# AroneyS/galah

Measured on AMD Instinct MI355X. Metric: precluster genome-pairs/sec at 10k genomes (s=1000) + sketch Gbases/s, higher is better.
Workload: dtype u64; 1 GPU; C3: 10000 synthetic genomes x 3000000 bp, clusters of 10, sub rate U(0,0.07), k=21, s=1000, min_ani=0.95; genomes=10000, genome_len=3000000, sketch_size=1000, k=21, parallelism=dp1, mode=lib

## Files before the change

galah_amd/csrc/api.cpp:

```cpp
#include <hip/hip_runtime.h>

#include <algorithm>
#include <chrono>
#include <cmath>
#include <cstdio>
#include <cstdlib>
#include <cstring>
#include <map>
#include <mutex>
#include <new>
#include <string>
#include <thread>
#include <vector>

#include "context.hpp"


namespace gg {

thread_local std::string g_thread_err;

void set_thread_error(const std::string& msg) { g_thread_err = msg; }

gg_status fail(gg_ctx* c, gg_status st, const std::string& msg) {
// ... 705 lines not shown
  b.border = n_old != 0;
  b.border0 = n_old;
  const char* re = getenv("GALAHGPU_INDEX_RANGE");
  const bool range_on = !(re && *re == '0');
  if (range_on && (r0 > 0 || r1 < n) && 5ull * (r1 - r0) <= 2ull * n) {
    uint32_t lg = 20;
    while (lg < 30 && (1ull << lg) < 16ull * (r1 - r0) * c->s) ++lg;
    b.bloom_log2 = lg;
    b.r0 = r0;
    b.r1 = r1;
    GG_HIP(c, scratch_t(c, "idx_bloom", (size_t)1 << (lg - 5), &b.bloom));
  }
  const char* be = getenv("GALAHGPU_INDEX_BUCKETS");
  b.bucket = !(be && *be == '0');
  if (b.bucket) {
    GG_HIP(c, scratch_t(c, "idx_hist", kIndexCoarse, &b.hist));
    GG_HIP(c, scratch_t(c, "idx_bbase", kIndexCoarse + 1, &b.bbase));
  }
  IndexLaunch a;
  a.sketches = d_sk;
  a.lens = d_lens;
  a.n = n;
  a.stride = c->s;
  a.kbits = kbits;
  a.row0 = r0;
  a.nb = nb;
  a.tile_begin = tb;
  a.tile_end = te;
  a.runinfo = b.runinfo;
  a.vals = b.keys_in;
  a.cmin = d_cmin;
  a.sufmin = d_sufmin;
  a.tmax = 2 * c->s;
  a.out = d_out;
  a.out_cap = cap;
  a.count = (unsigned long long*)d_count;
  a.border = n_old != 0;
  {
    const char* e = getenv("GALAHGPU_INDEX_MAX_SPLIT");
    a.max_split_log2 = e && *e ? (uint32_t)std::min(16, std::max(0, atoi(e))) : 16u;
  }
  a.overflow = b.flags + 2;
  {
    const char* e = getenv("GALAHGPU_INDEX_COST");
    const double k = !weigh_cost ? 0.0 : e && *e ? atof(e) : 0.0;
    const uint64_t n_new = n - n_old;
    const uint64_t npairs = n_old ? n_new * n_old + n_new * (n_new - 1) / 2 : pairs_in_tiles(n, tb, te);
    const double lim = k * (double)c->s * (double)npairs;
    a.cost = b.cost;
    a.cost_limit = k > 0 && lim < 1.8e19 ? (unsigned long long)lim : ~0ull;
  }
  uint64_t* d_count0;
  GG_HIP(c, scratch_t(c, "idx_count0", 1, &d_count0));
  GG_HIP(c, hipMemcpyAsync(d_count0, d_count, sizeof(uint64_t), hipMemcpyDeviceToDevice, st));
  auto launch_pairs = [&](bool guarded) -> gg_status {
    a.build_flags = guarded ? b.flags : nullptr;
    a.ents16 = b.bucket && index_ents16(n);
    GG_HIP(c, timed_launch(c, GG_KERNEL_PAIRS, work, st, [&] { return launch_index_pairs(a, r1 - r0, st); }));
    return GG_OK;
  };
  uint64_t info[2] = {0, 0};
  uint32_t kept = 0;
  uint32_t flags[4] = {0, 0, 0, 0};
  bool built = false, paired = false;
  if (b.bucket && !b.bloom) {
    const uint32_t nbb = index_bucket_bound(total);
    const char* se = getenv("GALAHGPU_INDEX_SPLIT");
    const bool split = !(se && *se == '0');
    if (split) {
      GG_HIP(c, scratch_t(c, "idx_split_cnt", (size_t)256 * n + 1, &b.split_cnt));
      GG_HIP(c, scratch_t(c, "idx_split_off", (size_t)256 * n + 1, &b.split_off));
      GG_HIP(c, scratch_t(c, "idx_split_hist", (size_t)256 * 16 * 256, &b.split_hist));
    }
    b.sort_tmp_bytes = split ? index_split_tmp_bytes(n) : index_bucket_sort_tmp_bytes(total);
    GG_HIP(c, scratch(c, "idx_sort_tmp", b.sort_tmp_bytes, &b.sort_tmp));
    GG_HIP(c, scratch_t(c, "idx_bstart", split ? (size_t)65537 : (size_t)nbb + 1, &b.bstart));
    GG_HIP(c, timed_launch(c, GG_KERNEL_PAIRS_INDEX, total, st, [&] { return index_fill(b, st); }));
    GG_HIP(c, timed_launch(c, GG_KERNEL_PAIRS_INDEX, 0, st, [&] { return index_build_buckets(b, total, nbb, st); }));
    gg_status ps = launch_pairs(true);
    if (ps != GG_OK) return ps;
    uint64_t* h_if;
    GG_HIP(c, host_scratch_t(c, "idx_info", 5, &h_if));
    GG_HIP(c, hipMemcpyAsync(h_if, b.info, 5 * sizeof(uint64_t), hipMemcpyDeviceToHost, st));
    GG_HIP(c, hipStreamSynchronize(st));
    memcpy(info, h_if, sizeof info);
    memcpy(flags, h_if + 2, sizeof flags);
    built = paired = flags[3] == 0;
    if (built && !flags[0] && h_if[4] > a.cost_limit) {
      *costly = true;
      return GG_OK;
    }
  } else {
    uint32_t nbuckets = 0;
    GG_HIP(c, timed_launch(c, GG_KERNEL_PAIRS_INDEX, total, st, [&] { return index_fill(b, st); }));
    GG_HIP(c, hipMemcpyAsync(info, b.info, sizeof info, hipMemcpyDeviceToHost, st));
    if (b.bloom) GG_HIP(c, hipMemcpyAsync(&kept, b.flags + 1, sizeof kept, hipMemcpyDeviceToHost, st));
    if (b.bucket)
      GG_HIP(c, hipMemcpyAsync(&nbuckets, b.bbase + kIndexCoarse, sizeof nbuckets, hipMemcpyDeviceToHost, st));
    GG_HIP(c, hipStreamSynchronize(st));
    if (b.bucket) {
      b.sort_tmp_bytes = index_bucket_sort_tmp_bytes(kept);
      GG_HIP(c, scratch(c, "idx_sort_tmp", b.sort_tmp_bytes, &b.sort_tmp));
      GG_HIP(c, scratch_t(c, "idx_bstart", (size_t)nbuckets + 1, &b.bstart));
      GG_HIP(c, timed_launch(c, GG_KERNEL_PAIRS_INDEX, 0, st,
                             [&] { return index_build_buckets(b, kept, nbuckets, st); }));
      GG_HIP(c, hipMemcpyAsync(flags, b.flags, sizeof flags, hipMemcpyDeviceToHost, st));
      GG_HIP(c, hipStreamSynchronize(st));
// ... 745 lines not shown
```

galah_amd/csrc/gg_internal.hpp:

```cpp
#pragma once

#include <hip/hip_runtime.h>

#include <cstdint>
#include <memory>
#include <string>
#include <vector>

#include "../../include/galahgpu.h"

namespace gg {

constexpr uint64_t kEmpty = ~0ull;

enum SketchStatus : uint32_t {
  kSketchOk = 0,
  kSketchRetryLarger = 1,
  kSketchRetrySmaller = 2,
  kSketchRetrySet = 3,
};

constexpr uint32_t kFlagOverflow = 1u;
constexpr uint32_t kFlagSawMax = 2u;
constexpr uint32_t kFlagSetMode = 4u;
// ... 232 lines not shown
  const uint64_t* file_text;
  const uint64_t* unit_len;
  const uint64_t* unit_pad;
  const uint32_t* unit_lane;
  uint32_t n_lanes, n_units;
  uint8_t* text;
  uint16_t* sym;
  uint32_t* flags;
  uint64_t* prof = nullptr;
};
constexpr uint16_t kSymPtr = 0x8000u;
struct GzMember {
  uint64_t off = 0, len = 0;
  uint32_t isize = 0, crc = 0;
};
struct InflateFile {
  uint64_t data_off = 0, data_len = 0;
  uint32_t isize = 0, crc = 0;
  bool gz = false;
  std::vector<GzMember> members;
};
bool bgzf_members(const uint8_t* buf, uint64_t n, uint64_t base, std::vector<GzMember>& out);
uint64_t bgzf_member_size(const uint8_t* b, uint64_t n);
bool gzip_member(const uint8_t* buf, size_t n, size_t* data_off, size_t* data_len, uint32_t* isize, uint32_t* crc);
bool gzip_header(const uint8_t* buf, size_t n, uint64_t file_size, size_t* data_off);
hipError_t launch_inflate_search(const InflateSearch& a, hipStream_t st);
hipError_t launch_slot_upload(uint8_t* dst, const uint8_t* src_mapped, uint64_t bytes, hipStream_t st);
hipError_t launch_inflate_decode(const InflateDecode& a, hipStream_t st);
hipError_t launch_inflate_expand(const InflatePlace& a, hipStream_t st);
hipError_t launch_inflate_resolve(const InflatePlace& a, hipStream_t st);
constexpr uint32_t kInflateCrcSeg = 4096;
hipError_t launch_inflate_crc(const uint8_t* text, uint32_t n_files, const uint64_t* file_text, const uint64_t* file_len,
                              const uint32_t* seg_first, uint32_t n_segs, uint32_t* seg_crc, uint32_t* crc,
                              hipStream_t st);

struct IndexBuild {
  const uint64_t* sketches;
  const uint32_t* lens;
  uint32_t n;
  uint32_t stride;
  uint32_t kbits;
  uint32_t max_run;
  uint64_t* offs;
  uint64_t* info;
  uint32_t* keys_in;
  uint32_t* keys_out;
  uint64_t* vals_in;
  uint64_t* vals_out;
  uint64_t* runinfo;
  uint32_t* mixed;
  void* sort_tmp;
  size_t sort_tmp_bytes;
  uint32_t* flags;
  unsigned long long* cost;
  uint32_t* bloom = nullptr;
  uint32_t bloom_log2 = 0;
  uint32_t r0 = 0, r1 = 0;
  bool bucket = false;
  uint32_t* hist = nullptr;
  uint32_t* bbase = nullptr;
  uint32_t* bstart = nullptr;
  uint32_t* split_cnt = nullptr;
  uint32_t* split_off = nullptr;
  uint32_t* split_hist = nullptr;
  bool border = false;
  uint32_t border0 = 0;
};
struct IndexLaunch {
  const uint64_t* sketches;
  const uint32_t* lens;
  uint32_t n;
  uint32_t stride;
  uint32_t kbits;
  uint32_t row0;
  uint32_t n_rows;
  uint64_t nb;
  uint64_t tile_begin;
  uint64_t tile_end;
  const uint64_t* runinfo;
  const uint32_t* vals;
  const uint32_t* cmin;
  const uint32_t* sufmin;
  uint32_t tmax;
  gg_pair* out;
  uint64_t out_cap;
  unsigned long long* count;
  uint32_t max_split_log2;
  uint32_t* overflow;
  const uint32_t* build_flags = nullptr;
  bool ents16 = false;
  const unsigned long long* cost = nullptr;
  unsigned long long cost_limit = ~0ull;
  bool big_map = false;
  bool border = false;
};
hipError_t index_fill(const IndexBuild& b, hipStream_t st);
hipError_t index_build(const IndexBuild& b, uint64_t total, uint32_t sh, uint32_t end_bit, hipStream_t st);
hipError_t index_build_buckets(const IndexBuild& b, uint64_t total, uint32_t nb_bound, hipStream_t st);
uint32_t index_bucket_bound(uint64_t entries);
size_t index_cost_bytes();
size_t index_sort_tmp_bytes(uint64_t total, uint32_t end_bit);
size_t index_bucket_sort_tmp_bytes(uint64_t total);
size_t index_split_tmp_bytes(uint32_t n);
constexpr uint32_t kIndexCoarse = 4096;
hipError_t launch_index_pairs(const IndexLaunch& a, uint32_t n_rows, hipStream_t st);
bool index_ents16(uint32_t n);
// ... 60 lines not shown
```

galah_amd/csrc/pairs_index.hip:

```cpp
#include <hipcub/hipcub.hpp>

#include <algorithm>

#include "device_util.hpp"
#include "gg_internal.hpp"

namespace gg {
namespace {

constexpr int kRowThreads = 256;
constexpr int kScanThreads = 1024;
constexpr uint32_t kXcds = 8;

struct KeyShape {
  uint32_t sh, norm;
};
__device__ __forceinline__ KeyShape key_shape(unsigned long long maxh) {
  const uint32_t bits = maxh ? 64u - (uint32_t)__builtin_clzll(maxh) : 0u;
  const uint32_t sh = bits > 32 ? bits - 32 : 0u;
  const uint32_t eb = bits - sh > 1u ? bits - sh : 1u;
  return KeyShape{sh, 32u - eb};
}

constexpr uint32_t kCoarseBits = 12;
constexpr uint32_t kBucketPad = 0xFFFFu;
constexpr uint32_t kBucketKeyBits = 16;
constexpr uint32_t kCoarse = 1u << kCoarseBits;
__device__ __forceinline__ uint32_t bucket_of(uint64_t h, KeyShape ks, const uint32_t* __restrict__ bbase) {
  const uint32_t key = (uint32_t)(h >> ks.sh) << ks.norm;
  const uint32_t c = key >> (32 - kCoarseBits);
  const uint32_t rel = key & ((1u << (32 - kCoarseBits)) - 1u);
  const uint32_t b0 = bbase[c], ns = bbase[c + 1] - b0;
  return b0 + (uint32_t)(((uint64_t)rel * ns) >> (32 - kCoarseBits));
}

__device__ __forceinline__ uint32_t count_le(const uint64_t* __restrict__ a, uint32_t n, uint64_t x) {
  uint32_t lo = 0, hi = n;
  while (lo < hi) {
    const uint32_t mid = (lo + hi) >> 1;
    if (a[mid] <= x) lo = mid + 1;
    else hi = mid;
  }
  return lo;
}

__global__ __launch_bounds__(kScanThreads) void index_scan_kernel(const uint64_t* __restrict__ sk,
                                                                  const uint32_t* __restrict__ lens, uint32_t n,
                                                                  uint32_t stride, uint64_t* __restrict__ offs,
                                                                  unsigned long long* __restrict__ info) {
  __shared__ unsigned long long wsum[kScanThreads / 64], wmax[kScanThreads / 64];
  const uint32_t tid = threadIdx.x;
  const uint32_t per = (n + kScanThreads - 1) / kScanThreads;
  const uint32_t b0 = min(tid * per, n), b1 = min(b0 + per, n);
  unsigned long long sum = 0, mx = 0;
  for (uint32_t i = b0; i < b1; ++i) {
    const uint32_t l = lens[i];
    sum += l;
    if (l) mx = max(mx, (unsigned long long)sk[(uint64_t)i * stride + l - 1]);
  }
  unsigned long long inc = sum;
  for (int o = 1; o < 64; o <<= 1) {
    const unsigned long long y = __shfl_up(inc, o);
    if ((tid & 63) >= (uint32_t)o) inc += y;
  }
  for (int o = 32; o > 0; o >>= 1) mx = max(mx, (unsigned long long)__shfl_xor(mx, o));
  if ((tid & 63) == 63) wsum[tid >> 6] = inc;
  if ((tid & 63) == 0) wmax[tid >> 6] = mx;
  __syncthreads();
  unsigned long long run = inc - sum;
  for (uint32_t w = 0; w < (tid >> 6); ++w) run += wsum[w];
  for (uint32_t i = b0; i < b1; ++i) {
    offs[i] = run;
    run += lens[i];
  }
  if (tid == kScanThreads - 1) {
    info[0] = run;
    unsigned long long m = 0;
    for (int w = 0; w < kScanThreads / 64; ++w) m = max(m, wmax[w]);
    info[1] = m;
  }
}

template <bool BUCKET>
__global__ __launch_bounds__(256) void index_fill_kernel(const uint64_t* __restrict__ sk,
                                                         const uint32_t* __restrict__ lens,
                                                         const uint64_t* __restrict__ offs, uint32_t n,
                                                         uint32_t stride, uint32_t kbits, uint32_t sh,
                                                         const unsigned long long* __restrict__ info,
                                                         const uint32_t* __restrict__ bbase,
                                                         uint32_t* __restrict__ keys, uint64_t* __restrict__ vals) {
  const KeyShape ks = BUCKET ? key_shape(info[1]) : KeyShape{sh, 0u};
  for (uint32_t i = blockIdx.x; i < n; i += gridDim.x) {
    const uint32_t len = lens[i];
    const uint64_t* row = sk + (uint64_t)i * stride;
    if (BUCKET) {
      const uint64_t o = (uint64_t)i * stride;
      for (uint32_t k = threadIdx.x; k < stride; k += 256) {
        ((uint16_t*)keys)[o + k] = (uint16_t)(k < len ? bucket_of(row[k], ks, bbase) : kBucketPad);
        ((uint32_t*)vals)[o + k] = (i << kbits) | k;
      }
      continue;
    }
    const uint64_t o = offs[i];
    for (uint32_t k = threadIdx.x; k < len; k += 256) {
// ... 735 lines not shown
      uint32_t rk = rank[r];
      bool sorted_run = false;
      if (g >= 2 && g <= kRowSortedRun) {
        const uint32_t row = e >> kbits;
        rk = 0;
        for (uint32_t x = 0; x < g; ++x) rk += (grp[start + x] >> kbits) < row ? 1u : 0u;
        sorted_run = true;
      }
      if (ents16) ((uint16_t*)ents)[lo + start + rk] = (uint16_t)(e >> kbits);
      else ents[lo + start + rk] = e;
      if (g > max_run) {
        atomicOr(&flags[0], 1u);
        continue;
      }
      if (BEFORE) {
        const uint32_t cnt = g < 2 ? 0u : sorted_run ? rk : g;
        runinfo[(uint64_t)(e >> kbits) * stride + (e & kmask)] = run_reads((uint64_t)lo + start, cnt);
        if ((e >> kbits) >= border0) {
          reads += cnt;
          gmax = max(gmax, g);
        }
        continue;
      }
      const uint32_t cnt = g < 2 ? 0u : sorted_run ? g - 1u - rk : g;
      runinfo[(uint64_t)(e >> kbits) * stride + (e & kmask)] =
          run_reads((uint64_t)lo + start + (sorted_run ? rk + 1u : 0u), cnt);
      reads += cnt;
      gmax = max(gmax, g);
    }
  }
  cost_add(cost, reads, gmax);
}

__device__ __forceinline__ void row_columns(uint32_t i, uint32_t n, uint64_t nb, uint64_t tb, uint64_t te,
                                            uint32_t& jlo, uint32_t& jhi) {
  const uint64_t I = i / GG_PAIR_TILE;
  const uint64_t rs = I * nb - I * (I - 1) / 2;
  const uint64_t t0 = rs, t1 = rs + (nb - I);
  const uint64_t a = max(t0, tb), b = min(t1, te);
  if (a >= b) {
    jlo = jhi = 0;
    return;
  }
  const uint64_t J0 = I + (a - rs), J1 = I + (b - rs);
  jlo = (uint32_t)max<uint64_t>(J0 * GG_PAIR_TILE, (uint64_t)i + 1);
  jhi = (uint32_t)min<uint64_t>(J1 * GG_PAIR_TILE, (uint64_t)n);
}

__device__ __forceinline__ uint32_t part_of(uint32_t j, uint32_t plog2) {
  return plog2 ? (j * 0x9E3779B1u) >> (32 - plog2) : 0u;
}

constexpr uint32_t kMemberLoads = 8;
template <bool E16, uint32_t MAPLOG2, bool BORDER = false>
__global__ __launch_bounds__(kRowThreads) void index_pairs_kernel(IndexLaunch a) {
  constexpr uint32_t kMapLog2 = MAPLOG2, kMap = 1u << kMapLog2, kMapFull = kMap * 3 / 4;
  __shared__ uint32_t mkey[kMap];
  __shared__ uint32_t mcnt[kMap];
  __shared__ uint32_t fill;
  __shared__ volatile uint32_t over;
  const uint32_t tid = threadIdx.x;
  const uint32_t per_xcd = (a.n_rows + kXcds - 1) / kXcds;
  const uint32_t ri_ = (blockIdx.x % kXcds) * per_xcd + blockIdx.x / kXcds;
  if (ri_ >= a.n_rows) return;
  const uint32_t i = a.row0 + ri_;
  if (i >= a.n) return;
  if (a.build_flags && ((a.build_flags[0] | a.build_flags[3]) || (a.cost && *a.cost > a.cost_limit))) return;
  uint32_t jlo, jhi;
  if (BORDER) jlo = 0u, jhi = i;
  else row_columns(i, a.n, a.nb, a.tile_begin, a.tile_end, jlo, jhi);
  const uint32_t la = a.lens[i];
  if (jlo >= jhi || la == 0) return;
  const uint64_t* ri = a.runinfo + (uint64_t)i * a.stride;
  const uint64_t* A = a.sketches + (uint64_t)i * a.stride;
  const uint64_t xa = A[la - 1];
  uint32_t plog2 = 0;
  for (uint32_t p = 0; p < (1u << plog2);) {
    for (uint32_t x = tid; x < kMap; x += kRowThreads) mkey[x] = 0u, mcnt[x] = 0u;
    if (tid == 0) fill = 0u, over = 0u;
    __syncthreads();
    uint64_t info_next = tid < la ? ri[tid] : 0ull;
    for (uint32_t k = tid; k < la; k += kRowThreads) {
      if (over) break;
      const uint64_t info = info_next;
      info_next = k + kRowThreads < la ? ri[k + kRowThreads] : 0ull;
      const uint32_t cnt = (uint32_t)(info >> 32);
      if (cnt == 0) continue;
      const uint32_t q_first = (uint32_t)info, end = q_first + cnt;
      bool stop = false;
      for (uint32_t q0 = q_first; q0 < end && !stop; q0 += kMemberLoads) {
        uint32_t jv[kMemberLoads];
#pragma unroll
        for (uint32_t u = 0; u < kMemberLoads; ++u) {
          const uint32_t q = q0 + u;
          jv[u] = q < end ? (E16 ? (uint32_t)((const uint16_t*)a.vals)[q] : a.vals[q] >> a.kbits) : jhi;
        }
#pragma unroll
        for (uint32_t u = 0; u < kMemberLoads; ++u) {
          const uint32_t j = jv[u];
          if (stop || j < jlo || j >= jhi) continue;
          if (plog2 && part_of(j, plog2) != p) continue;
          uint32_t h = (j * 0x85EBCA6Bu) >> (32 - kMapLog2);
          for (uint32_t probe = 0;; ++probe) {
            const uint32_t old = atomicCAS(&mkey[h], 0u, j + 1u);
            if (old == 0u) {
              if (atomicAdd(&fill, 1u) >= kMapFull) over = 1u;
            }
            if (old == 0u || old == j + 1u) {
              atomicAdd(&mcnt[h], 1u);
              break;
            }
            if (probe >= kMap) {
              over = 1u;
              break;
            }
            h = (h + 1) & (kMap - 1);
          }
          if (over) stop = true;
        }
      }
      if (stop) break;
    }
    __syncthreads();
    if (over) {
      if (plog2 < a.max_split_log2) {
        ++plog2;
        p *= 2;
        __syncthreads();
        continue;
      }
      if (tid == 0) atomicOr(a.overflow, 1u);
      return;
    }
    for (uint32_t x = tid; x < kMap; x += kRowThreads) {
      const uint32_t key = mkey[x];
      if (!key) continue;
      const uint32_t j = key - 1u, common = mcnt[x];
      const uint32_t lb = a.lens[j];
      if (common < a.sufmin[min(la, lb)]) continue;
      const uint64_t* B = a.sketches + (uint64_t)j * a.stride;
      const uint64_t xb = B[lb - 1];
      const uint32_t total = xa <= xb ? la + count_le(B, lb, xa) - common : count_le(A, la, xb) + lb - common;
      if (total <= a.tmax && common >= a.cmin[total]) {
        const unsigned long long slot = atomicAdd(a.count, 1ull);
        if (slot < a.out_cap) a.out[slot] = BORDER ? gg_pair{j, i, common, total} : gg_pair{i, j, common, total};
      }
    }
    __syncthreads();
    ++p;
  }
}

}

static bool hist_sampling() {
  const char* e = getenv("GALAHGPU_INDEX_HIST_SAMPLE");
  return !(e && *e == '0');
}

hipError_t index_fill(const IndexBuild& b, hipStream_t st) {
  hipError_t e = hipMemsetAsync(b.flags, 0, 4 * sizeof(uint32_t) + index_cost_bytes(), st);
  if (e != hipSuccess) return e;
  hipLaunchKernelGGL(index_scan_kernel, dim3(1), dim3(kScanThreads), 0, st, b.sketches, b.lens, b.n, b.stride,
                     b.offs, (unsigned long long*)b.info);
  e = hipGetLastError();
  if (e != hipSuccess) return e;
  const unsigned long long* info = (const unsigned long long*)b.info;
  if (b.bucket) {
    e = hipMemsetAsync(b.hist, 0, kCoarse * sizeof(uint32_t), st);
    if (e != hipSuccess) return e;
    hipLaunchKernelGGL(bucket_hist_kernel, dim3(std::max(1u, std::min<uint32_t>(b.n, 1024))), dim3(256), 0, st,
                       b.sketches, b.lens, b.n, b.stride, info, b.hist, hist_sampling() ? 1u : 0u);
    hipLaunchKernelGGL(bucket_base_kernel, dim3(1), dim3(kBaseThreads), 0, st, b.hist, info, b.bbase);
    e = hipGetLastError();
    if (e != hipSuccess) return e;
  }
  if (!b.bloom) return hipSuccess;
  e = hipMemsetAsync(b.bloom, 0, ((size_t)1 << b.bloom_log2) / 8, st);
  if (e != hipSuccess) return e;
  if (b.r1 > b.r0)
    hipLaunchKernelGGL(bloom_build_kernel, dim3(std::min<uint32_t>(b.r1 - b.r0, 16384)), dim3(256), 0, st,
                       b.sketches, b.lens, b.r0, b.r1, b.stride, b.bloom, b.bloom_log2);
  const dim3 grid(std::max(1u, std::min<uint32_t>(b.n, 4096)));
  if (b.bucket)
    hipLaunchKernelGGL(index_fill_range_kernel<true>, grid, dim3(256), 0, st, b.sketches, b.lens, b.n, b.stride,
                       b.kbits, b.bloom, b.bloom_log2, b.r0, b.r1, info, b.bbase, b.flags + 1, b.keys_in, b.vals_in);
  else
    hipLaunchKernelGGL(index_fill_range_kernel<false>, grid, dim3(256), 0, st, b.sketches, b.lens, b.n, b.stride,
                       b.kbits, b.bloom, b.bloom_log2, b.r0, b.r1, info, nullptr, b.flags + 1, b.keys_in,
                       b.vals_in);
  return hipGetLastError();
}

hipError_t index_build(const IndexBuild& b, uint64_t total, uint32_t sh, uint32_t end_bit, hipStream_t st) {
  if (total == 0) return hipSuccess;
  if (!b.bloom)
    hipLaunchKernelGGL(index_fill_kernel<false>, dim3(std::min<uint32_t>(b.n, 16384)), dim3(256), 0, st,
                       b.sketches, b.lens, b.offs, b.n, b.stride, b.kbits, sh, nullptr, nullptr, b.keys_in,
                       b.vals_in);
  hipError_t e = hipGetLastError();
  if (e != hipSuccess) return e;
  size_t bytes = b.sort_tmp_bytes;
  e = hipcub::DeviceRadixSort::SortPairs(b.sort_tmp, bytes, b.keys_in, b.keys_out, b.vals_in, b.vals_out,
                                         (int)total, 0, (int)end_bit, st);
  if (e != hipSuccess) return e;
  e = hipMemsetAsync(b.mixed, 0, ((total + 31) / 32) * sizeof(uint32_t), st);
  if (e != hipSuccess) return e;
  const uint64_t waves = (total + 63) / 64;
  const uint32_t blocks = (uint32_t)(std::min<uint64_t>(8192, std::max<uint64_t>(1, (waves + 4 * kXcds - 1) /
                                                                                  (4 * kXcds))) * kXcds);
  const uint32_t rows_ordered = b.bloom ? 0u : 1u;
  if (b.border)
    hipLaunchKernelGGL(index_runs_kernel<true>, dim3(blocks), dim3(256), 0, st, b.keys_out, b.vals_out, total,
                       b.stride, b.kbits, b.max_run, b.runinfo, b.keys_in, b.mixed, b.flags, rows_ordered, b.cost,
                       b.border0);
  else
    hipLaunchKernelGGL(index_runs_kernel<false>, dim3(blocks), dim3(256), 0, st, b.keys_out, b.vals_out, total,
                       b.stride, b.kbits, b.max_run, b.runinfo, b.keys_in, b.mixed, b.flags, rows_ordered, b.cost, 0u);
  e = hipGetLastError();
  if (e != hipSuccess) return e;
  const uint64_t words = (total + 31) / 32;
  const dim3 mixed_grid((uint32_t)std::min<uint64_t>(4096, (words + 255) / 256));
  if (b.border)
    hipLaunchKernelGGL(index_mixed_kernel<true>, mixed_grid, dim3(256), 0, st, b.keys_out, b.vals_out, total, b.stride,
                       b.kbits, b.mixed, b.runinfo, b.keys_in);
  else
    hipLaunchKernelGGL(index_mixed_kernel<false>, mixed_grid, dim3(256), 0, st, b.keys_out, b.vals_out, total,
                       b.stride, b.kbits, b.mixed, b.runinfo, b.keys_in);
  e = hipGetLastError();
  if (e != hipSuccess) return e;
  hipLaunchKernelGGL(index_cost_sum_kernel, dim3(1), dim3(kCostSlots), 0, st, b.cost);
  return hipGetLastError();
}

size_t index_cost_bytes() { return (size_t)(1 + kCostSlots) * kCostStride * sizeof(unsigned long long); }

static hipError_t index_sort_buckets(const IndexBuild& b, uint64_t total, uint32_t nb_bound, hipStream_t st);

hipError_t index_build_buckets(const IndexBuild& b, uint64_t total, uint32_t nb_bound, hipStream_t st) {
  if (total == 0 || nb_bound == 0) return hipSuccess;
  const uint32_t* nbuckets_d = b.bbase + kCoarse;
  uint32_t* vout = (uint32_t*)b.vals_out;
  if (b.split_cnt && !b.bloom) {
    const dim3 rows((b.n + kXcds - 1) / kXcds * kXcds);
    hipLaunchKernelGGL(split_keys_kernel, rows, dim3(256), 0, st, b.sketches, b.lens, b.n, b.stride,
                       (const unsigned long long*)b.info, b.bbase, (uint16_t*)b.keys_in, b.split_cnt);
    hipError_t e = hipGetLastError();
    if (e != hipSuccess) return e;
    size_t bytes = b.sort_tmp_bytes;
    e = hipcub::DeviceScan::ExclusiveSum(b.sort_tmp, bytes, b.split_cnt, b.split_off, (int)(kSuper * b.n + 1), st);
    if (e != hipSuccess) return e;
    hipLaunchKernelGGL(split_scatter_kernel, rows, dim3(256), 0, st, (const uint16_t*)b.keys_in, b.lens, b.n,
                       b.stride, b.kbits, b.split_cnt, b.split_off, (uint8_t*)b.keys_out, (uint32_t*)b.vals_in);
    const uint32_t parts = (uint32_t)std::max<uint64_t>(
        1, std::min<uint64_t>(kSuperParts, total / ((uint64_t)kSuper * 3 * kPlaceChunk / 2)));
    hipLaunchKernelGGL(superbin_count_kernel, dim3(kSuper * parts), dim3(256), 0, st, (const uint8_t*)b.keys_out,
                       b.split_off, b.n, parts, b.split_hist);
    hipLaunchKernelGGL(superbin_place_kernel, dim3(kSuper * parts), dim3(kPlaceThreads), 0, st,
                       (const uint8_t*)b.keys_out, (const uint32_t*)b.vals_in, b.split_off, b.n, parts, b.split_hist,
                       b.bstart, vout);
    e = hipGetLastError();
    if (e != hipSuccess) return e;
  } else {
    hipError_t e = index_sort_buckets(b, total, nb_bound, st);
    if (e != hipSuccess) return e;
  }
  const uint32_t per_xcd = (nb_bound + kXcds - 1) / kXcds;
  const char* bt = getenv("GALAHGPU_BUCKET_THREADS");
  const int threads = bt && *bt ? atoi(bt) : 1024;
  auto go = [&](auto kern, int t) {
    hipLaunchKernelGGL(kern, dim3(per_xcd * kXcds), dim3(t), 0, st, vout, b.bstart, nbuckets_d, total, b.sketches,
                       b.stride, b.kbits, b.max_run, b.runinfo, b.keys_in, index_ents16(b.n) ? 1u : 0u, b.flags,
                       b.cost, b.border ? b.border0 : 0u);
  };
  if (b.border) {
    if (threads == 256) go(index_bucket_kernel<256, true>, 256);
    else if (threads == 512) go(index_bucket_kernel<512, true>, 512);
    else go(index_bucket_kernel<1024, true>, 1024);
  } else if (threads == 256) go(index_bucket_kernel<256, false>, 256);
  else if (threads == 512) go(index_bucket_kernel<512, false>, 512);
  else go(index_bucket_kernel<1024, false>, 1024);
  hipError_t e2 = hipGetLastError();
  if (e2 != hipSuccess) return e2;
  hipLaunchKernelGGL(index_cost_sum_kernel, dim3(1), dim3(kCostSlots), 0, st, b.cost);
  return hipGetLastError();
}

static hipError_t index_sort_buckets(const IndexBuild& b, uint64_t total, uint32_t nb_bound, hipStream_t st) {
  const uint32_t* nbuckets_d = b.bbase + kCoarse;
  if (!b.bloom)
    hipLaunchKernelGGL(index_fill_kernel<true>, dim3(std::min<uint32_t>(b.n, 16384)), dim3(256), 0, st, b.sketches,
                       b.lens, nullptr, b.n, b.stride, b.kbits, 0u, (const unsigned long long*)b.info, b.bbase,
                       b.keys_in, b.vals_in);
  hipError_t e = hipGetLastError();
  if (e != hipSuccess) return e;
  uint32_t* vin = (uint32_t*)b.vals_in;
  uint32_t* vout = (uint32_t*)b.vals_out;
  size_t bytes = b.sort_tmp_bytes;
  e = hipcub::DeviceRadixSort::SortPairs(b.sort_tmp, bytes, (const uint16_t*)b.keys_in, (uint16_t*)b.keys_out, vin,
                                         vout, (int)total, 0, (int)kBucketKeyBits, st);
  if (e != hipSuccess) return e;
  e = hipMemsetAsync(b.bstart, 0xFF, ((size_t)nb_bound + 1) * sizeof(uint32_t), st);
  if (e != hipSuccess) return e;
  hipLaunchKernelGGL(bucket_bounds_kernel, dim3((uint32_t)std::min<uint64_t>(16384, total / 2048 + 1)), dim3(256), 0,
                     st, (const uint16_t*)b.keys_out, total, nbuckets_d, b.bstart);
  return hipGetLastError();
}

size_t index_split_tmp_bytes(uint32_t n) {
  size_t bytes = 0;
  (void)hipcub::DeviceScan::ExclusiveSum(nullptr, bytes, (const uint32_t*)nullptr, (uint32_t*)nullptr,
                                         (int)(kSuper * n + 1));
  return bytes;
}

uint32_t index_bucket_bound(uint64_t entries) {
  return (uint32_t)std::min<uint64_t>(kBucketPad - 1, entries / 1024 + kCoarse);
}

size_t index_sort_tmp_bytes(uint64_t total, uint32_t end_bit) {
  size_t bytes = 0;
  (void)hipcub::DeviceRadixSort::SortPairs(nullptr, bytes, (const uint32_t*)nullptr, (uint32_t*)nullptr,
                                           (const uint64_t*)nullptr, (uint64_t*)nullptr, (int)total, 0, (int)end_bit);
  return bytes;
}

size_t index_bucket_sort_tmp_bytes(uint64_t total) {
  size_t bytes = 0;
  (void)hipcub::DeviceRadixSort::SortPairs(nullptr, bytes, (const uint16_t*)nullptr, (uint16_t*)nullptr,
                                           (const uint32_t*)nullptr, (uint32_t*)nullptr, (int)total, 0,
                                           (int)kBucketKeyBits);
  return bytes;
}

hipError_t launch_index_pairs(const IndexLaunch& a, uint32_t n_rows, hipStream_t st) {
  if (n_rows == 0) return hipSuccess;
  IndexLaunch b = a;
  b.n_rows = n_rows;
  const dim3 grid((n_rows + kXcds - 1) / kXcds * kXcds);
  if (a.border) {
    if (a.ents16) {
      if (a.big_map) hipLaunchKernelGGL((index_pairs_kernel<true, 13, true>), grid, dim3(kRowThreads), 0, st, b);
      else hipLaunchKernelGGL((index_pairs_kernel<true, 11, true>), grid, dim3(kRowThreads), 0, st, b);
    } else {
      if (a.big_map) hipLaunchKernelGGL((index_pairs_kernel<false, 13, true>), grid, dim3(kRowThreads), 0, st, b);
      else hipLaunchKernelGGL((index_pairs_kernel<false, 11, true>), grid, dim3(kRowThreads), 0, st, b);
    }
  } else if (a.ents16) {
    if (a.big_map) hipLaunchKernelGGL((index_pairs_kernel<true, 13>), grid, dim3(kRowThreads), 0, st, b);
    else hipLaunchKernelGGL((index_pairs_kernel<true, 11>), grid, dim3(kRowThreads), 0, st, b);
  } else {
    if (a.big_map) hipLaunchKernelGGL((index_pairs_kernel<false, 13>), grid, dim3(kRowThreads), 0, st, b);
    else hipLaunchKernelGGL((index_pairs_kernel<false, 11>), grid, dim3(kRowThreads), 0, st, b);
  }
  return hipGetLastError();
}

namespace {
__global__ __launch_bounds__(256) void pair_keys_kernel(const gg_pair* __restrict__ p, uint32_t cnt, uint32_t n,
                                                        uint64_t* __restrict__ keys, uint32_t* __restrict__ idx) {
  for (uint32_t x = blockIdx.x * 256 + threadIdx.x; x < cnt; x += gridDim.x * 256) {
    const gg_pair q = p[x];
    keys[x] = (uint64_t)q.i * n + q.j;
    idx[x] = x;
  }
}

__global__ __launch_bounds__(256) void pair_gather_kernel(const gg_pair* __restrict__ p, uint32_t cnt,
                                                          const uint32_t* __restrict__ idx,
                                                          gg_pair* __restrict__ sorted) {
  for (uint32_t y = blockIdx.x * 256 + threadIdx.x; y < cnt; y += gridDim.x * 256) sorted[y] = p[idx[y]];
}
}

uint32_t pair_key_bits(uint32_t n) {
  const uint64_t mx = (uint64_t)n * n;
  uint32_t bits = 1;
  while (bits < 64 && (mx >> bits) != 0) ++bits;
  return bits;
}

size_t pair_sort_tmp_bytes(uint64_t cnt, uint32_t n) {
  size_t bytes = 0;
  (void)hipcub::DeviceRadixSort::SortPairs(nullptr, bytes, (const uint64_t*)nullptr, (uint64_t*)nullptr,
                                           (const uint32_t*)nullptr, (uint32_t*)nullptr, (int)cnt, 0,
                                           (int)pair_key_bits(n));
  return bytes;
}

hipError_t sort_pairs_device(const gg_pair* d_pairs, uint64_t cnt, uint32_t n, uint64_t* keys, uint64_t* keys_out,
                             uint32_t* idx, uint32_t* idx_out, gg_pair* sorted, void* tmp, size_t tmp_bytes,
                             hipStream_t st) {
  if (cnt == 0) return hipSuccess;
  if (cnt >= (1ull << 31)) return hipErrorInvalidValue;
  const dim3 grid((uint32_t)std::min<uint64_t>(4096, (cnt + 255) / 256));
  hipLaunchKernelGGL(pair_keys_kernel, grid, dim3(256), 0, st, d_pairs, (uint32_t)cnt, n, keys, idx);
  hipError_t e = hipGetLastError();
  if (e != hipSuccess) return e;
  e = hipcub::DeviceRadixSort::SortPairs(tmp, tmp_bytes, keys, keys_out, idx, idx_out, (int)cnt, 0,
                                         (int)pair_key_bits(n), st);
  if (e != hipSuccess) return e;
  hipLaunchKernelGGL(pair_gather_kernel, grid, dim3(256), 0, st, d_pairs, (uint32_t)cnt, idx_out, sorted);
  return hipGetLastError();
}

bool index_ents16(uint32_t n) { return n <= 65536u; }
// ... 3 lines not shown
```

galah_amd/csrc/sketch.hip:

```cpp
#include "device_util.hpp"
#include "gg_internal.hpp"
#include "sketch_core.hpp"

namespace gg {
namespace {

constexpr int kGroup = 4;
constexpr int kBlock = 256;
#ifndef GG_K1_MIN_WAVES
#define GG_K1_MIN_WAVES 7
#endif
#ifndef GG_K1_STRETCH
#define GG_K1_STRETCH 2
#endif
constexpr int kStretch = GG_K1_STRETCH;
static_assert(kStretch >= 1 && kStretch <= 16, "stretch");

template <int R>
__device__ __forceinline__ uint64_t rotl64(uint64_t x) {
  uint32_t lo = (uint32_t)x, hi = (uint32_t)(x >> 32);
  if (R >= 32) {
    const uint32_t t = lo;
    lo = hi;
    hi = t;
// ... 445 lines not shown
      }
    }
  };
  if (bad && *bad != ~0ull) {
    finish(~0u, setm);
    return;
  }
  if (f & kFlagOverflow) {
    finish(setm ? kSketchRetrySmaller : kSketchRetrySet, true);
    return;
  }
  const uint32_t NB = 1u << nb_log2;
  const uint64_t t = tau[slot];
  const uint32_t tbits = 64 - __builtin_clzll(t | 1ull);
  const uint32_t shift = tbits > nb_log2 ? tbits - nb_log2 : 0u;
  auto scan = [&](bool hi) -> uint32_t {
    const uint32_t per = (NB + T - 1) / T;
    const uint32_t b0 = min(tid * per, NB), b1 = min(b0 + per, NB);
    uint32_t sum = 0;
    for (uint32_t b = b0; b < b1; ++b) sum += hi ? cnt[b] >> 16 : cnt[b] & 0xFFFFu;
    uint32_t inc = sum;
    for (int o = 1; o < 64; o <<= 1) {
      const uint32_t y = __shfl_up(inc, o);
      if ((tid & 63) >= (uint32_t)o) inc += y;
    }
    if ((tid & 63) == 63) wsum[tid >> 6] = inc;
    __syncthreads();
    uint32_t run = inc - sum;
    for (uint32_t w = 0; w < (tid >> 6); ++w) run += wsum[w];
    uint32_t total = 0;
    for (uint32_t w = 0; w < (T + 63) / 64; ++w) total += wsum[w];
    for (uint32_t b = b0; b < b1; ++b) {
      const uint32_t c = cnt[b];
      if (hi) {
        cnt[b] = (c & 0xFFFFu) | (run << 16);
        run += c >> 16;
      } else {
        cnt[b] = run;
        run += c;
      }
    }
    __syncthreads();
    return total;
  };
  uint32_t n;
  for (uint32_t i = tid; i < NB; i += T) cnt[i] = 0;
  if (!setm) {
    n = listed;
    if (n > sort_pow2) {
      finish(kSketchRetrySet, true);
      return;
    }
    constexpr uint32_t kListV = 8;
    auto list_pass = [&](auto&& fn) {
      for (uint32_t i0 = tid * kListV; i0 < n; i0 += T * kListV) {
        uint64_t v[kListV];
#pragma unroll
        for (uint32_t j = 0; j < kListV; j += 2) {
          if (i0 + j + 1 < n) {
            const ulonglong2 p = *(const ulonglong2*)(tab + i0 + j);
            v[j] = p.x;
            v[j + 1] = p.y;
          } else if (i0 + j < n) {
            v[j] = tab[i0 + j];
          }
        }
#pragma unroll
        for (uint32_t j = 0; j < kListV; ++j)
          if (i0 + j < n) fn(v[j]);
      }
    };
    __syncthreads();
    list_pass([&](uint64_t v) { atomicAdd(&cnt[(uint32_t)(v >> shift)], 1u); });
    __syncthreads();
    scan(false);
    list_pass([&](uint64_t v) { buf[atomicAdd(&cnt[(uint32_t)(v >> shift)], 1u)] = v; });
    __syncthreads();
  } else {
    if (tid == 0) fill = 0;
    __syncthreads();
    constexpr uint32_t kGatherV = 8;
    const uint32_t steps = (cap + T * kGatherV - 1) / (T * kGatherV);
    for (uint32_t it = 0; it < steps; ++it) {
      const uint32_t i0 = (it * T + tid) * kGatherV;
      uint64_t v[kGatherV];
#pragma unroll
      for (uint32_t j = 0; j < kGatherV; j += 2) {
        if (i0 + j < cap) {
          const ulonglong2 p = *(const ulonglong2*)(tab + i0 + j);
          v[j] = p.x;
          v[j + 1] = p.y;
        } else {
          v[j] = v[j + 1] = kEmpty;
        }
      }
      uint32_t c = 0;
#pragma unroll
      for (uint32_t j = 0; j < kGatherV; ++j) c += v[j] != kEmpty ? 1u : 0u;
      uint32_t inc = c;
      for (int o = 1; o < 64; o <<= 1) {
        const uint32_t y = __shfl_up(inc, o);
        if (lane >= (uint32_t)o) inc += y;
      }
      uint32_t base = 0;
      if (lane == 63 && inc) base = atomicAdd(&fill, inc);
      uint32_t at = __shfl(base, 63) + inc - c;
#pragma unroll
      for (uint32_t j = 0; j < kGatherV; ++j) {
        if (v[j] != kEmpty) {
          if (at < sort_pow2) buf[at] = v[j];
          ++at;
        }
      }
    }
    __syncthreads();
    n = fill;
    if (n > sort_pow2) {
      finish(kSketchRetrySmaller, true);
      return;
    }
    for (uint32_t e = tid; e < n; e += T) atomicAdd(&cnt[(uint32_t)(buf[e] >> shift)], 1u);
    __syncthreads();
    scan(false);
    for (uint32_t e = tid; e < n; e += T) {
      const uint64_t v = buf[e];
      tab[atomicAdd(&cnt[(uint32_t)(v >> shift)], 1u)] = v;
    }
    __syncthreads();
    for (uint32_t e0 = tid; e0 < n; e0 += 4 * T) {
// ... 137 lines not shown
```

Baseline: 1.147 billion genome-pairs/s.

## Add wave-per-row short pairs kernel and fold memsets into scan kernel

Adds a pairs kernel that gives each row its own wave with a small per-wave hash map when the sketch stride is small. Rows that overflow that map fall back to the full workgroup path. The flag, hist and count zeroing and the count copy move into the scan kernel, which removes several memset and memcpy launches. Bucket threads default to 512 for small totals, and the sketch list pass keeps loaded values in registers across the two passes when they fit. The short kernel risks extra work and serialised fallback for rows with many partners.

```diff
diff --git a/galah_amd/csrc/api.cpp b/galah_amd/csrc/api.cpp
--- a/galah_amd/csrc/api.cpp
+++ b/galah_amd/csrc/api.cpp
@@ -781,7 +781,8 @@
   }
   uint64_t* d_count0;
   GG_HIP(c, scratch_t(c, "idx_count0", 1, &d_count0));
-  GG_HIP(c, hipMemcpyAsync(d_count0, d_count, sizeof(uint64_t), hipMemcpyDeviceToDevice, st));
+  b.count = d_count;
+  b.count0 = d_count0;
   auto launch_pairs = [&](bool guarded) -> gg_status {
     a.build_flags = guarded ? b.flags : nullptr;
     a.ents16 = b.bucket && index_ents16(n);
diff --git a/galah_amd/csrc/gg_internal.hpp b/galah_amd/csrc/gg_internal.hpp
--- a/galah_amd/csrc/gg_internal.hpp
+++ b/galah_amd/csrc/gg_internal.hpp
@@ -308,6 +308,8 @@
   void* sort_tmp;
   size_t sort_tmp_bytes;
   uint32_t* flags;
+  const uint64_t* count = nullptr;
+  uint64_t* count0 = nullptr;
   unsigned long long* cost;
   uint32_t* bloom = nullptr;
   uint32_t bloom_log2 = 0;
diff --git a/galah_amd/csrc/pairs_index.hip b/galah_amd/csrc/pairs_index.hip
--- a/galah_amd/csrc/pairs_index.hip
+++ b/galah_amd/csrc/pairs_index.hip
@@ -47,9 +47,17 @@
 __global__ __launch_bounds__(kScanThreads) void index_scan_kernel(const uint64_t* __restrict__ sk,
                                                                   const uint32_t* __restrict__ lens, uint32_t n,
                                                                   uint32_t stride, uint64_t* __restrict__ offs,
-                                                                  unsigned long long* __restrict__ info) {
+                                                                  unsigned long long* __restrict__ info,
+                                                                  unsigned long long* __restrict__ zero,
+                                                                  uint32_t n_zero, uint32_t* __restrict__ hist,
+                                                                  const uint64_t* __restrict__ count,
+                                                                  uint64_t* __restrict__ count0) {
   __shared__ unsigned long long wsum[kScanThreads / 64], wmax[kScanThreads / 64];
   const uint32_t tid = threadIdx.x;
+  for (uint32_t x = tid; x < n_zero; x += kScanThreads) zero[x] = 0ull;
+  if (hist)
+    for (uint32_t x = tid; x < kCoarse; x += kScanThreads) hist[x] = 0u;
+  if (count0 && tid == 0) *count0 = *count;
   const uint32_t per = (n + kScanThreads - 1) / kScanThreads;
   const uint32_t b0 = min(tid * per, n), b1 = min(b0 + per, n);
   unsigned long long sum = 0, mx = 0;
@@ -891,20 +899,83 @@
 }
 
 constexpr uint32_t kMemberLoads = 8;
-template <bool E16, uint32_t MAPLOG2, bool BORDER = false>
-__global__ __launch_bounds__(kRowThreads) void index_pairs_kernel(IndexLaunch a) {
-  constexpr uint32_t kMapLog2 = MAPLOG2, kMap = 1u << kMapLog2, kMapFull = kMap * 3 / 4;
-  __shared__ uint32_t mkey[kMap];
-  __shared__ uint32_t mcnt[kMap];
-  __shared__ uint32_t fill;
-  __shared__ volatile uint32_t over;
+
+template <bool E16, uint32_t MAPLOG2, uint32_t THREADS>
+__device__ __forceinline__ void count_partners(const IndexLaunch& a, const uint64_t* __restrict__ ri, uint32_t la,
+                                               uint32_t jlo, uint32_t jhi, uint32_t plog2, uint32_t p,
+                                               uint32_t* mkey, uint32_t* mcnt, uint32_t* fill,
+                                               volatile uint32_t* over, uint32_t t) {
+  constexpr uint32_t kMap = 1u << MAPLOG2, kMapFull = kMap * 3 / 4;
+  uint64_t info_next = t < la ? ri[t] : 0ull;
+  for (uint32_t k = t; k < la; k += THREADS) {
+    if (*over) break;
+    const uint64_t info = info_next;
+    info_next = k + THREADS < la ? ri[k + THREADS] : 0ull;
+    const uint32_t cnt = (uint32_t)(info >> 32);
+    if (cnt == 0) continue;
+    const uint32_t q_first = (uint32_t)info, end = q_first + cnt;
+    bool stop = false;
+    for (uint32_t q0 = q_first; q0 < end && !stop; q0 += kMemberLoads) {
+      uint32_t jv[kMemberLoads];
+#pragma unroll
+      for (uint32_t u = 0; u < kMemberLoads; ++u) {
+        const uint32_t q = q0 + u;
+        jv[u] = q < end ? (E16 ? (uint32_t)((const uint16_t*)a.vals)[q] : a.vals[q] >> a.kbits) : jhi;
+      }
+#pragma unroll
+      for (uint32_t u = 0; u < kMemberLoads; ++u) {
+        const uint32_t j = jv[u];
+        if (stop || j < jlo || j >= jhi) continue;
+        if (plog2 && part_of(j, plog2) != p) continue;
+        uint32_t h = (j * 0x85EBCA6Bu) >> (32 - MAPLOG2);
+        for (uint32_t probe = 0;; ++probe) {
+          const uint32_t old = atomicCAS(&mkey[h], 0u, j + 1u);
+          if (old == 0u) {
+            if (atomicAdd(fill, 1u) >= kMapFull) *over = 1u;
+          }
+          if (old == 0u || old == j + 1u) {
+            atomicAdd(&mcnt[h], 1u);
+            break;
+          }
+          if (probe >= kMap) {
+            *over = 1u;
+            break;
+          }
+          h = (h + 1) & (kMap - 1);
+        }
+        if (*over) stop = true;
+      }
+    }
+    if (stop) break;
+  }
+}
+
+template <uint32_t MAPLOG2, uint32_t THREADS, bool BORDER>
+__device__ __forceinline__ void emit_partners(const IndexLaunch& a, uint32_t i, uint32_t la,
+                                              const uint64_t* __restrict__ A, uint64_t xa, const uint32_t* mkey,
+                                              const uint32_t* mcnt, uint32_t t) {
+  constexpr uint32_t kMap = 1u << MAPLOG2;
+  for (uint32_t x = t; x < kMap; x += THREADS) {
+    const uint32_t key = mkey[x];
+    if (!key) continue;
+    const uint32_t j = key - 1u, common = mcnt[x];
+    const uint32_t lb = a.lens[j];
+    if (common < a.sufmin[min(la, lb)]) continue;
+    const uint64_t* B = a.sketches + (uint64_t)j * a.stride;
+    const uint64_t xb = B[lb - 1];
+    const uint32_t total = xa <= xb ? la + count_le(B, lb, xa) - common : count_le(A, la, xb) + lb - common;
+    if (total <= a.tmax && common >= a.cmin[total]) {
+      const unsigned long long slot = atomicAdd(a.count, 1ull);
+      if (slot < a.out_cap) a.out[slot] = BORDER ? gg_pair{j, i, common, total} : gg_pair{i, j, common, total};
+    }
+  }
+}
+
+template <bool E16, uint32_t MAPLOG2, bool BORDER>
+__device__ __forceinline__ void row_pairs_workgroup(const IndexLaunch& a, uint32_t i, uint32_t* mkey, uint32_t* mcnt,
+                                                    uint32_t* fill, volatile uint32_t* over) {
+  constexpr uint32_t kMap = 1u << MAPLOG2;
   const uint32_t tid = threadIdx.x;
-  const uint32_t per_xcd = (a.n_rows + kXcds - 1) / kXcds;
-  const uint32_t ri_ = (blockIdx.x % kXcds) * per_xcd + blockIdx.x / kXcds;
-  if (ri_ >= a.n_rows) return;
-  const uint32_t i = a.row0 + ri_;
-  if (i >= a.n) return;
-  if (a.build_flags && ((a.build_flags[0] | a.build_flags[3]) || (a.cost && *a.cost > a.cost_limit))) return;
   uint32_t jlo, jhi;
   if (BORDER) jlo = 0u, jhi = i;
   else row_columns(i, a.n, a.nb, a.tile_begin, a.tile_end, jlo, jhi);
@@ -916,78 +987,84 @@
   uint32_t plog2 = 0;
   for (uint32_t p = 0; p < (1u << plog2);) {
     for (uint32_t x = tid; x < kMap; x += kRowThreads) mkey[x] = 0u, mcnt[x] = 0u;
-    if (tid == 0) fill = 0u, over = 0u;
+    if (tid == 0) *fill = 0u, *over = 0u;
     __syncthreads();
-    uint64_t info_next = tid < la ? ri[tid] : 0ull;
-    for (uint32_t k = tid; k < la; k += kRowThreads) {
-      if (over) break;
-      const uint64_t info = info_next;
-      info_next = k + kRowThreads < la ? ri[k + kRowThreads] : 0ull;
-      const uint32_t cnt = (uint32_t)(info >> 32);
-      if (cnt == 0) continue;
-      const uint32_t q_first = (uint32_t)info, end = q_first + cnt;
-      bool stop = false;
-      for (uint32_t q0 = q_first; q0 < end && !stop; q0 += kMemberLoads) {
-        uint32_t jv[kMemberLoads];
-#pragma unroll
-        for (uint32_t u = 0; u < kMemberLoads; ++u) {
-          const uint32_t q = q0 + u;
-          jv[u] = q < end ? (E16 ? (uint32_t)((const uint16_t*)a.vals)[q] : a.vals[q] >> a.kbits) : jhi;
-        }
-#pragma unroll
-        for (uint32_t u = 0; u < kMemberLoads; ++u) {
-          const uint32_t j = jv[u];
-          if (stop || j < jlo || j >= jhi) continue;
-          if (plog2 && part_of(j, plog2) != p) continue;
-          uint32_t h = (j * 0x85EBCA6Bu) >> (32 - kMapLog2);
-          for (uint32_t probe = 0;; ++probe) {
-            const uint32_t old = atomicCAS(&mkey[h], 0u, j + 1u);
-            if (old == 0u) {
-              if (atomicAdd(&fill, 1u) >= kMapFull) over = 1u;
-            }
-            if (old == 0u || old == j + 1u) {
-              atomicAdd(&mcnt[h], 1u);
-              break;
-            }
-            if (probe >= kMap) {
-              over = 1u;
-              break;
-            }
-            h = (h + 1) & (kMap - 1);
-          }
-          if (over) stop = true;
-        }
-      }
-      if (stop) break;
-    }
+    count_partners<E16, MAPLOG2, kRowThreads>(a, ri, la, jlo, jhi, plog2, p, mkey, mcnt, fill, over, tid);
     __syncthreads();
-    if (over) {
+    if (*over) {
+      __syncthreads();
       if (plog2 < a.max_split_log2) {
         ++plog2;
         p *= 2;
-        __syncthreads();
         continue;
       }
       if (tid == 0) atomicOr(a.overflow, 1u);
       return;
     }
-    for (uint32_t x = tid; x < kMap; x += kRowThreads) {
-      const uint32_t key = mkey[x];
-      if (!key) continue;
-      const uint32_t j = key - 1u, common = mcnt[x];
-      const uint32_t lb = a.lens[j];
-      if (common < a.sufmin[min(la, lb)]) continue;
-      const uint64_t* B = a.sketches + (uint64_t)j * a.stride;
-      const uint64_t xb = B[lb - 1];
-      const uint32_t total = xa <= xb ? la + count_le(B, lb, xa) - common : count_le(A, la, xb) + lb - common;
-      if (total <= a.tmax && common >= a.cmin[total]) {
-        const unsigned long long slot = atomicAdd(a.count, 1ull);
-        if (slot < a.out_cap) a.out[slot] = BORDER ? gg_pair{j, i, common, total} : gg_pair{i, j, common, total};
-      }
-    }
+    emit_partners<MAPLOG2, kRowThreads, BORDER>(a, i, la, A, xa, mkey, mcnt, tid);
     __syncthreads();
     ++p;
   }
+}
+
+template <bool E16, uint32_t MAPLOG2, bool BORDER = false>
+__global__ __launch_bounds__(kRowThreads) void index_pairs_kernel(IndexLaunch a) {
+  constexpr uint32_t kMap = 1u << MAPLOG2;
+  __shared__ uint32_t mkey[kMap];
+  __shared__ uint32_t mcnt[kMap];
+  __shared__ uint32_t fill;
+  __shared__ volatile uint32_t over;
+  const uint32_t per_xcd = (a.n_rows + kXcds - 1) / kXcds;
+  const uint32_t ri_ = (blockIdx.x % kXcds) * per_xcd + blockIdx.x / kXcds;
+  if (ri_ >= a.n_rows) return;
+  const uint32_t i = a.row0 + ri_;
+  if (i >= a.n) return;
+  if (a.build_flags && ((a.build_flags[0] | a.build_flags[3]) || (a.cost && *a.cost > a.cost_limit))) return;
+  row_pairs_workgroup<E16, MAPLOG2, BORDER>(a, i, mkey, mcnt, &fill, &over);
+}
+
+constexpr uint32_t kShortRows = kRowThreads / 64;
+constexpr uint32_t kShortStride = 2048;
+constexpr uint32_t kShortMapLog2 = 8, kShortMap = 1u << kShortMapLog2;
+static_assert(kShortRows * kShortMap <= (1u << 11), "the waves' maps lie in the workgroup's");
+
+template <bool E16>
+__global__ __launch_bounds__(kRowThreads) void index_pairs_short_kernel(IndexLaunch a) {
+  constexpr uint32_t kMapLog2 = 11, kMap = 1u << kMapLog2;
+  __shared__ uint32_t mkey[kMap];
+  __shared__ uint32_t mcnt[kMap];
+  __shared__ uint32_t fill;
+  __shared__ volatile uint32_t over;
+  __shared__ uint32_t wfill[kShortRows];
+  __shared__ volatile uint32_t wover[kShortRows];
+  const uint32_t tid = threadIdx.x, lane = tid & 63, wave = tid >> 6;
+  const uint32_t groups = (a.n_rows + kShortRows - 1) / kShortRows;
+  const uint32_t per_xcd = (groups + kXcds - 1) / kXcds;
+  const uint32_t g = (blockIdx.x % kXcds) * per_xcd + blockIdx.x / kXcds;
+  if (blockIdx.x / kXcds >= per_xcd || g >= groups) return;
+  if (a.build_flags && ((a.build_flags[0] | a.build_flags[3]) || (a.cost && *a.cost > a.cost_limit))) return;
+  const uint32_t ri_ = g * kShortRows + wave;
+  const uint32_t i = a.row0 + ri_;
+  uint32_t jlo = 0, jhi = 0, la = 0;
+  if (ri_ < a.n_rows && i < a.n) {
+    row_columns(i, a.n, a.nb, a.tile_begin, a.tile_end, jlo, jhi);
+    la = a.lens[i];
+  }
+  const bool live = jlo < jhi && la != 0;
+  uint32_t* wkey = mkey + wave * kShortMap;
+  uint32_t* wcnt = mcnt + wave * kShortMap;
+  for (uint32_t x = lane; x < kShortMap; x += 64) wkey[x] = 0u, wcnt[x] = 0u;
+  if (lane == 0) wfill[wave] = 0u, wover[wave] = 0u;
+  __syncthreads();
+  const uint64_t* A = a.sketches + (uint64_t)i * a.stride;
+  if (live)
+    count_partners<E16, kShortMapLog2, 64>(a, a.runinfo + (uint64_t)i * a.stride, la, jlo, jhi, 0u, 0u, wkey, wcnt,
+                                           &wfill[wave], &wover[wave], lane);
+  __syncthreads();
+  if (live && !wover[wave]) emit_partners<kShortMapLog2, 64, false>(a, i, la, A, A[la - 1], wkey, wcnt, lane);
+  __syncthreads();
+  for (uint32_t w = 0; w < kShortRows; ++w)
+    if (wover[w]) row_pairs_workgroup<E16, kMapLog2, false>(a, a.row0 + g * kShortRows + w, mkey, mcnt, &fill, &over);
 }
 
 }
@@ -998,16 +1075,15 @@
 }
 
 hipError_t index_fill(const IndexBuild& b, hipStream_t st) {
-  hipError_t e = hipMemsetAsync(b.flags, 0, 4 * sizeof(uint32_t) + index_cost_bytes(), st);
-  if (e != hipSuccess) return e;
+  static_assert(4 * sizeof(uint32_t) % sizeof(unsigned long long) == 0, "flags: whole 8-byte words");
+  const uint32_t n_zero = (uint32_t)((4 * sizeof(uint32_t) + index_cost_bytes()) / sizeof(unsigned long long));
   hipLaunchKernelGGL(index_scan_kernel, dim3(1), dim3(kScanThreads), 0, st, b.sketches, b.lens, b.n, b.stride,
-                     b.offs, (unsigned long long*)b.info);
-  e = hipGetLastError();
+                     b.offs, (unsigned long long*)b.info, (unsigned long long*)b.flags, n_zero,
+                     b.bucket ? b.hist : nullptr, b.count, b.count ? b.count0 : nullptr);
+  hipError_t e = hipGetLastError();
   if (e != hipSuccess) return e;
   const unsigned long long* info = (const unsigned long long*)b.info;
   if (b.bucket) {
-    e = hipMemsetAsync(b.hist, 0, kCoarse * sizeof(uint32_t), st);
-    if (e != hipSuccess) return e;
     hipLaunchKernelGGL(bucket_hist_kernel, dim3(std::max(1u, std::min<uint32_t>(b.n, 1024))), dim3(256), 0, st,
                        b.sketches, b.lens, b.n, b.stride, info, b.hist, hist_sampling() ? 1u : 0u);
     hipLaunchKernelGGL(bucket_base_kernel, dim3(1), dim3(kBaseThreads), 0, st, b.hist, info, b.bbase);
@@ -1106,7 +1182,7 @@
   }
   const uint32_t per_xcd = (nb_bound + kXcds - 1) / kXcds;
   const char* bt = getenv("GALAHGPU_BUCKET_THREADS");
-  const int threads = bt && *bt ? atoi(bt) : 1024;
+  const int threads = bt && *bt ? atoi(bt) : (total + 59999) / 60000 <= 1024 ? 512 : 1024;
   auto go = [&](auto kern, int t) {
     hipLaunchKernelGGL(kern, dim3(per_xcd * kXcds), dim3(t), 0, st, vout, b.bstart, nbuckets_d, total, b.sketches,
                        b.stride, b.kbits, b.max_run, b.runinfo, b.keys_in, index_ents16(b.n) ? 1u : 0u, b.flags,
@@ -1185,12 +1261,16 @@
       if (a.big_map) hipLaunchKernelGGL((index_pairs_kernel<false, 13, true>), grid, dim3(kRowThreads), 0, st, b);
       else hipLaunchKernelGGL((index_pairs_kernel<false, 11, true>), grid, dim3(kRowThreads), 0, st, b);
     }
-  } else if (a.ents16) {
-    if (a.big_map) hipLaunchKernelGGL((index_pairs_kernel<true, 13>), grid, dim3(kRowThreads), 0, st, b);
-    else hipLaunchKernelGGL((index_pairs_kernel<true, 11>), grid, dim3(kRowThreads), 0, st, b);
+  } else if (a.big_map) {
+    if (a.ents16) hipLaunchKernelGGL((index_pairs_kernel<true, 13>), grid, dim3(kRowThreads), 0, st, b);
+    else hipLaunchKernelGGL((index_pairs_kernel<false, 13>), grid, dim3(kRowThreads), 0, st, b);
+  } else if (a.stride > kShortStride) {
+    if (a.ents16) hipLaunchKernelGGL((index_pairs_kernel<true, 11>), grid, dim3(kRowThreads), 0, st, b);
+    else hipLaunchKernelGGL((index_pairs_kernel<false, 11>), grid, dim3(kRowThreads), 0, st, b);
   } else {
-    if (a.big_map) hipLaunchKernelGGL((index_pairs_kernel<false, 13>), grid, dim3(kRowThreads), 0, st, b);
-    else hipLaunchKernelGGL((index_pairs_kernel<false, 11>), grid, dim3(kRowThreads), 0, st, b);
+    const dim3 short_grid(((n_rows + kShortRows - 1) / kShortRows + kXcds - 1) / kXcds * kXcds);
+    if (a.ents16) hipLaunchKernelGGL(index_pairs_short_kernel<true>, short_grid, dim3(kRowThreads), 0, st, b);
+    else hipLaunchKernelGGL(index_pairs_short_kernel<false>, short_grid, dim3(kRowThreads), 0, st, b);
   }
   return hipGetLastError();
 }
diff --git a/galah_amd/csrc/sketch.hip b/galah_amd/csrc/sketch.hip
--- a/galah_amd/csrc/sketch.hip
+++ b/galah_amd/csrc/sketch.hip
@@ -521,29 +521,49 @@
       return;
     }
     constexpr uint32_t kListV = 8;
+    auto load_list = [&](uint64_t (&v)[kListV], uint32_t i0) {
+#pragma unroll
+      for (uint32_t j = 0; j < kListV; j += 2) {
+        v[j] = v[j + 1] = 0ull;
+        if (i0 + j + 1 < n) {
+          const ulonglong2 p = *(const ulonglong2*)(tab + i0 + j);
+          v[j] = p.x;
+          v[j + 1] = p.y;
+        } else if (i0 + j < n) {
+          v[j] = tab[i0 + j];
+        }
+      }
+    };
     auto list_pass = [&](auto&& fn) {
       for (uint32_t i0 = tid * kListV; i0 < n; i0 += T * kListV) {
         uint64_t v[kListV];
-#pragma unroll
-        for (uint32_t j = 0; j < kListV; j += 2) {
-          if (i0 + j + 1 < n) {
-            const ulonglong2 p = *(const ulonglong2*)(tab + i0 + j);
-            v[j] = p.x;
-            v[j + 1] = p.y;
-          } else if (i0 + j < n) {
-            v[j] = tab[i0 + j];
-          }
-        }
+        load_list(v, i0);
 #pragma unroll
         for (uint32_t j = 0; j < kListV; ++j)
           if (i0 + j < n) fn(v[j]);
       }
     };
-    __syncthreads();
-    list_pass([&](uint64_t v) { atomicAdd(&cnt[(uint32_t)(v >> shift)], 1u); });
-    __syncthreads();
-    scan(false);
-    list_pass([&](uint64_t v) { buf[atomicAdd(&cnt[(uint32_t)(v >> shift)], 1u)] = v; });
+    auto add = [&](uint64_t x) { atomicAdd(&cnt[(uint32_t)(x >> shift)], 1u); };
+    auto place = [&](uint64_t x) { buf[atomicAdd(&cnt[(uint32_t)(x >> shift)], 1u)] = x; };
+    __syncthreads();
+    if (n <= T * kListV) {
+      const uint32_t i0 = tid * kListV;
+      uint64_t v[kListV];
+      load_list(v, i0);
+#pragma unroll
+      for (uint32_t j = 0; j < kListV; ++j)
+        if (i0 + j < n) add(v[j]);
+      __syncthreads();
+      scan(false);
+#pragma unroll
+      for (uint32_t j = 0; j < kListV; ++j)
+        if (i0 + j < n) place(v[j]);
+    } else {
+      list_pass(add);
+      __syncthreads();
+      scan(false);
+      list_pass(place);
+    }
     __syncthreads();
   } else {
     if (tid == 0) fill = 0;
```

New measurement: 1.145 billion genome-pairs/s. No clear change (-0.2%).
